# pscoro/JPEG-XL-Lossy-Image-Compression-Thesis

Hardware: AMD Instinct MI355X
Metric: MPix/s VarDCT encode @ d1.0, 8K RGB (higher is better)
Workload: dtype f32; 1 GPU; 8k 7680x4320 RGB8 (synth_rgb8), VarDCT d1 e7, cjxl defaults (JXG_FLAGS_CJXL_DEFAULTS: Gaborish + EPF + masking AQ), proposals=0, ans-coded, 1 frame(s) per step, 2 distinct frames cycled, streaming entry points (jxg_submit_rgb8_device / jxg_receive, one host thread); global_batch=1, parallelism=frame-dp1

## Files before the change

jpeg-xl-lossy-image-compression-thesis_amd/csrc/jxg_merge.hip:

```cpp
#include <float.h>

#include <cstdio>
#include <type_traits>

#include "jxg_device.h"
#include "jxg_kernels.h"
#include "jxg_lee_tables.h"

namespace jxg {

__constant__ float c_llf_p[4 * 8];
__constant__ float c_llf_ib[4 * 64];

constexpr int kMThreads = 256;
#ifndef JXG_MERGE_WPE
#define JXG_MERGE_WPE 4
#endif
#ifndef JXG_MERGE_WRITE_WPE
#define JXG_MERGE_WRITE_WPE 3
#endif
constexpr int kMS = 65;
constexpr int kMPlane = 64 * kMS;

template <int N>
constexpr int ilog2c() {
  return N <= 1 ? 0 : 1 + ilog2c<N / 2>();
}

typedef float f2 __attribute__((ext_vector_type(2)));

template <int N, class T>
__device__ __forceinline__ void lee(T* x) {
  if constexpr (N > 1) {
    constexpr int h = N / 2, l = ilog2c<N>();
    T a[h], b[h];
#pragma unroll
    for (int i = 0; i < h; i++) {
      a[i] = x[i] + x[N - 1 - i];
      b[i] = (x[i] - x[N - 1 - i]) * kLeeC[l][i];
    }
    lee<h>(a);
    lee<h>(b);
#pragma unroll
    for (int k = 0; k < h; k++) x[2 * k] = a[k];
#pragma unroll
    for (int k = 0; k < h - 1; k++) x[2 * k + 1] = b[k] + b[k + 1];
    x[N - 1] = b[h - 1];
  }
}
template <int N>
__device__ __forceinline__ void dct_from(const float* src, int st, float* x) {
#pragma unroll
  for (int k = 0; k < N; k++) x[k] = src[k * st];
  lee<N>(x);
  constexpr int l = ilog2c<N>();
#pragma unroll
  for (int k = 0; k < N; k++) x[k] = x[k] * kLeeS[l][k];
}
template <int N, class T>
__device__ __forceinline__ T dctN_first(T xi, T xm, int i, int h) {
  return h == 0 ? xi + xm : (xi - xm) * kLeeC[ilog2c<N>()][i];
}
template <int N, class T, class Out>
__device__ __forceinline__ void dctN_rest(T* t, int h, Out out) {
  constexpr int l = ilog2c<N>(), H = N / 2;
  lee<H>(t);
  if (h == 0) {
#pragma unroll
    for (int k = 0; k < H; k++) out(k, t[k] * kLeeS[l][2 * k]);
  } else {
#pragma unroll
    for (int k = 0; k < H - 1; k++) out(k, (t[k] + t[k + 1]) * kLeeS[l][2 * k + 1]);
    out(H - 1, t[H - 1] * kLeeS[l][N - 1]);
  }
}
template <class T>
__device__ __forceinline__ T dct64_first(T xi, T xm, int i, int h) {
  return dctN_first<64>(xi, xm, i, h);
}
template <class T, class Out>
__device__ __forceinline__ void dct64_rest(T* t, int h, Out out) {
  dctN_rest<64>(t, h, out);
}

#ifdef JXG_MERGE_PROFILE
__device__ unsigned long long g_mprof[16][8];
#define MPROF_MARK(k)                                                 \
  do {                                                                \
    if (!WRITE && threadIdx.x == 0) {                                 \
      const unsigned long long now_ = __builtin_readcyclecounter();   \
      if ((k) > 0) atomicAdd(&g_mprof[P.si][(k)], now_ - mprof_t0);   \
      mprof_t0 = now_;                                                \
    }                                                                 \
  } while (0)
#else
#define MPROF_MARK(k) \
  do {                \
  } while (0)
#endif
#ifdef JXG_MERGE_PROFILE
__device__ unsigned long long g_mzero[3][2];
#define MZERO_COUNT(ch, hit)                                                          \
  do {                                                                                \
    if ((int)(threadIdx.x & 63) == __ffsll((unsigned long long)__ballot(1)) - 1) {    \
      atomicAdd(&g_mzero[(ch)][0], 1ull);                                             \
      if (hit) atomicAdd(&g_mzero[(ch)][1], 1ull);                                    \
    }                                                                                 \
  } while (0)
#else
#define MZERO_COUNT(ch, hit) \
  do {                       \
  } while (0)
#endif

struct ShapeDesc {
  int type, lcy, lcx;
  float tmul;
};
constexpr ShapeDesc kShapes[kNumShapes] = {
    {6, 1, 0, 1.0f},   {7, 0, 1, 1.0f},   {4, 1, 1, 1.0f},
    {10, 2, 1, 1.02f}, {11, 1, 2, 1.02f}, {5, 2, 2, 1.03f},
    {19, 3, 2, 1.05f}, {20, 2, 3, 1.05f}, {18, 3, 3, 1.05f}};

__device__ __forceinline__ int bitlen_u(uint32_t v) { return 32 - __clz(v); }

struct MergeLds {
  float co[2 * kMPlane];
  float llf[3][64];
  float qsum[3][4][32];
  float btab[256];
  float vr3[32][3];
  int vbits[32];
  int vnz[32][3];
  int vraw[32];
  int valid[32];
  uint8_t braw[64];
  int any;
};
struct WriteLds : MergeLds {
  uint32_t ssrc[32];
  uint32_t sgb[32];
  float skc[2][32];
};
template <class L>
constexpr bool kIsWrite = std::is_same<L, WriteLds>::value;
__device__ __forceinline__ float& llf_at(MergeLds& S, int c, int b) { return S.llf[c][b]; }
__device__ __forceinline__ int pass_src(int pass, int lc) { return pass ? 2 : 1 - lc; }
__device__ __forceinline__ int pass_plane(int pass, int lc) { return pass ? 1 : lc; }
__device__ __forceinline__ constexpr int chan_plane(int ch) { return ch == 1 ? 0 : 1; }

struct Pass {
  int si, type, lcy, lcx, soff, ls, tx, ty, tile;
  float tmul;
  __device__ __forceinline__ int cy() const { return 1 << lcy; }
  __device__ __forceinline__ int cx() const { return 1 << lcx; }
  __device__ __forceinline__ int R() const { return 8 << lcy; }
  __device__ __forceinline__ int C() const { return 8 << lcx; }
  __device__ __forceinline__ int lR() const { return 3 + lcy; }
  __device__ __forceinline__ int lC() const { return 3 + lcx; }
  __device__ __forceinline__ int lGX() const { return 3 - lcx; }
  __device__ __forceinline__ int lNV() const { return 6 - lcx - lcy; }
  __device__ __forceinline__ int NV() const { return 1 << lNV(); }
  __device__ __forceinline__ int bx0(int v) const { return (v & ((1 << lGX()) - 1)) << lcx; }
  __device__ __forceinline__ int by0(int v) const { return (v >> lGX()) << lcy; }
  __device__ __forceinline__ int off(int v, int plane) const {
    return plane * kMPlane + by0(v) * 8 * kMS + bx0(v) * 8;
  }
};

#ifndef JXG_MERGE_CHUNK
#define JXG_MERGE_CHUNK 32
#endif
__device__ __forceinline__ bool decode_wg(const MergeArgs& a, int& tile, int& si) {
  constexpr int T = JXG_MERGE_CHUNK;
  const int b = blockIdx.x, x = b & 7, q = b >> 3;
  const int r = q % (kNumShapes * T);
  si = r / T;
  tile = ((q / (kNumShapes * T)) * T + r % T) * 8 + x;
  if (tile >= (int)a.ntiles) return false;
  if (a.tile_list) tile = (int)a.tile_list[tile];
  return true;
}

__device__ __forceinline__ Pass make_pass(const MergeArgs& a, int tile, int si) {
  Pass P;
  P.si = si;
  const ShapeDesc& D = kShapes[si];
  P.type = D.type;
  P.lcy = D.lcy;
  P.lcx = D.lcx;
  P.tmul = D.tmul;
  P.soff = kShapeOff[si];
  P.ls = max(D.lcy, D.lcx);
  P.tile = tile;
  P.tx = tile % (int)a.tiles_x;
  P.ty = tile / (int)a.tiles_x;
  return P;
}

template <int C>
__device__ __forceinline__ void load_row(const float* src, float* d) {
#pragma unroll
  for (int q = 0; q < C / 4; q++) {
    const float4 u = reinterpret_cast<const float4*>(src)[q];
    d[4 * q] = u.x;
    d[4 * q + 1] = u.y;
    d[4 * q + 2] = u.z;
    d[4 * q + 3] = u.w;
  }
}
template <int C, int NCH, class L>
__device__ __forceinline__ void row_pass(const MergeArgs& a, const Pass& P, L& S, int pass) {
  constexpr bool WRITE = kIsWrite<L>;
  const float* tsrc = a.xyb + (size_t)P.tile * (3 * 4096);
  const int R = P.R(), lvr = P.lNV() + P.lR();
  if constexpr (C == 64) {
    const int npairs = NCH * P.NV() * R / 2;
    const int n = ((npairs + 63) >> 6) << 7;
    for (int i = threadIdx.x; i < n; i += kMThreads) {
      const int h = (i >> 6) & 1, pp = ((i >> 7) << 6) | (i & 63), r = pp * 2;
      if (pp >= npairs) continue;
      const int c = r >> lvr, v = (r >> P.lR()) & (P.NV() - 1), y = r & (R - 1);
      if (!S.valid[v]) continue;
      const float* src0;
      if constexpr (WRITE) src0 = a.xyb + S.ssrc[v] + pass_src(pass, c) * 4096 + y * 64;
      else src0 = tsrc + pass_src(pass, c) * 4096 + (P.by0(v) * 8 + y) * 64;
      const float4* s0 = reinterpret_cast<const float4*>(src0);
      const float4* s1 = s0 + 16;
      f2 t[32];
#pragma unroll
      for (int q = 0; q < 8; q++) {
        const float4 a0 = s0[q], b0 = s0[15 - q], a1 = s1[q], b1 = s1[15 - q];
        const float fa0[4] = {a0.x, a0.y, a0.z, a0.w}, fb0[4] = {b0.x, b0.y, b0.z, b0.w};
        const float fa1[4] = {a1.x, a1.y, a1.z, a1.w}, fb1[4] = {b1.x, b1.y, b1.z, b1.w};
#pragma unroll
        for (int j = 0; j < 4; j++)
          t[4 * q + j] = dct64_first(f2{fa0[j], fa1[j]}, f2{fb0[3 - j], fb1[3 - j]}, 4 * q + j, h);
      }
      const int off = P.off(v, pass_plane(pass, c)) + y * kMS;
      dct64_rest(t, h, [&](int k, f2 o) {
        S.co[off + 2 * k + h] = o.x;
        S.co[off + kMS + 2 * k + h] = o.y;
      });
    }
  } else {
    constexpr int PER = (NCH * 4096 / C + kMThreads - 1) / kMThreads;
    const int nrows = NCH * P.NV() * R;
    const int lgx = P.lGX();
    auto row_of = [&](int rr, int& c, int& v, int& y) {
      c = rr >> lvr;
      const int i = rr & ((1 << lvr) - 1);
      y = (i >> lgx) & (R - 1);
      v = ((i >> (lgx + P.lR())) << lgx) | (i & ((1 << lgx) - 1));
    };
    float buf[PER][C];
#pragma unroll
    for (int k = 0; k < PER; k++) {
      const int r = threadIdx.x + k * kMThreads;
      if (r < nrows) {
        int c, v, y;
        row_of(r, c, v, y);
        if constexpr (WRITE)
          load_row<C>(a.xyb + S.ssrc[v] + pass_src(pass, c) * 4096 + y * 64, buf[k]);
        else
          load_row<C>(tsrc + pass_src(pass, c) * 4096 + (P.by0(v) * 8 + y) * 64 + P.bx0(v) * 8,
                      buf[k]);
      } else {
#pragma unroll
        for (int q = 0; q < C; q++) buf[k][q] = 0.0f;
      }
    }
    constexpr int l = ilog2c<C>();
#pragma unroll
    for (int k = 0; k < PER; k += 2) {
      const int r0 = threadIdx.x + k * kMThreads, r1 = r0 + kMThreads;
      if (r0 >= nrows) continue;
      int c0, v0, y0, c1, v1, y1;
      row_of(r0, c0, v0, y0);
      row_of(r1, c1, v1, y1);
      const bool ok0 = S.valid[v0], ok1 = k + 1 < PER && r1 < nrows && S.valid[v1];
      if (!ok0 && !ok1) continue;
      if (k + 1 < PER) {
        f2 x[C];
#pragma unroll
        for (int q = 0; q < C; q++) x[q] = f2{buf[k][q], buf[k + 1][q]};
        lee<C>(x);
        const int off0 = P.off(v0, pass_plane(pass, c0)) + y0 * kMS,
                  off1 = P.off(v1, pass_plane(pass, c1)) + y1 * kMS;
#pragma unroll
        for (int q = 0; q < C; q++) {
          const f2 o = x[q] * kLeeS[l][q];
          if (ok0) S.co[off0 + q] = o.x;
          if (ok1) S.co[off1 + q] = o.y;
        }
      } else {
        float* x = buf[k];
        lee<C>(x);
        const int off0 = P.off(v0, pass_plane(pass, c0)) + y0 * kMS;
#pragma unroll
        for (int q = 0; q < C; q++) S.co[off0 + q] = x[q] * kLeeS[l][q];
      }
    }
  }
}

template <int R, int NCH>
__device__ __forceinline__ void col_pass(const Pass& P, MergeLds& S, int pass) {
  constexpr int lR = ilog2c<R>(), nb = 64 / R, lnb = 6 - lR;
  constexpr int npairs = NCH * nb * 32;
  const int lGX = P.lGX(), lC = P.lC();
  auto col_of = [&](int pidx, int& off, bool& okA, bool& okB) {
    const int X = pidx & 31, band = (pidx >> 5) & (nb - 1), c = pidx >> (5 + lnb);
    off = pass_plane(pass, c) * kMPlane + band * R * kMS + X;
    okA = S.valid[(band << lGX) | (X >> lC)];
    okB = S.valid[(band << lGX) | ((X + 32) >> lC)];
  };
  if constexpr (R == 64 || (R >= 16 && npairs <= kMThreads / 2)) {
    constexpr int H = R / 2;
    constexpr int n = ((npairs + 63) >> 6) << 7;
    for (int i0 = 0; i0 < n; i0 += kMThreads) {
      const int i = i0 + threadIdx.x;
      const int h = (i >> 6) & 1, p = ((i >> 7) << 6) | (i & 63);
      int off = 0;
      bool okA = false, okB = false;
      if (p < npairs) col_of(p, off, okA, okB);
      const bool act = okA || okB;
      f2 o[H];
      if (act) {
        const float* q0 = S.co + off;
        f2 t[H];
#pragma unroll
        for (int j = 0; j < H; j++)
          t[j] = dctN_first<R>(f2{q0[j * kMS], q0[j * kMS + 32]},
                               f2{q0[(R - 1 - j) * kMS], q0[(R - 1 - j) * kMS + 32]}, j, h);
        dctN_rest<R>(t, h, [&](int k, f2 u) { o[k] = u; });
      }
      __syncthreads();
      if (act) {
#pragma unroll
        for (int k = 0; k < H; k++) {
          if (okA) S.co[off + (2 * k + h) * kMS] = o[k].x;
          if (okB) S.co[off + 32 + (2 * k + h) * kMS] = o[k].y;
        }
      }
    }
  } else {
    for (int p = threadIdx.x; p < npairs; p += kMThreads) {
      int off;
      bool okA, okB;
      col_of(p, off, okA, okB);
      if (!okA && !okB) continue;
      float* col = S.co + off;
      f2 o[R];
#pragma unroll
      for (int k = 0; k < R; k++) o[k] = f2{col[k * kMS], col[k * kMS + 32]};
      lee<R>(o);
#pragma unroll
      for (int k = 0; k < R; k++) {
        const f2 u = o[k] * kLeeS[lR][k];
        if (okA) col[k * kMS] = u.x;
        if (okB) col[k * kMS + 32] = u.y;
      }
    }
  }
}

template <int N>
__device__ __forceinline__ void load_f(const float* p, float* d) {
#pragma unroll
  for (int i = 0; i < N / 4; i++) {
    const float4 v = reinterpret_cast<const float4*>(p)[i];
    d[4 * i] = v.x;
    d[4 * i + 1] = v.y;
    d[4 * i + 2] = v.z;
    d[4 * i + 3] = v.w;
  }
}
template <int RPC>
struct QTab {
  static constexpr int NIT = RPC == 8 ? 2 : 1;
  float w[NIT][RPC], sd[NIT][RPC], iw[NIT][RPC];
};
__device__ __forceinline__ int qtab_index(const Pass& P, int ky, int x) {
  return P.soff + ((ky >> 2) * P.C() + x) * 4;
}
template <int RPC, bool WRITE, int CH>
__device__ __forceinline__ void load_qtab(const MergeArgs& a, const Pass& P, QTab<RPC>& T) {
  constexpr int STOT = kShapeOff[kNumShapes];
#pragma unroll
  for (int it = 0; it < QTab<RPC>::NIT; it++) {
    const int j = threadIdx.x + it * kMThreads;
    const int ch = j >> (P.lNV() + P.lC()), x = j & (P.C() - 1);
#pragma unroll
    for (int kk = 0; kk < RPC; kk += 4) {
      const int ti = qtab_index(P, ch * RPC + kk, x);
      load_f<4>(a.wk + (size_t)CH * STOT + ti, &T.w[it][kk]);
      if (!WRITE) load_f<4>(a.sdk + (size_t)CH * STOT + ti, &T.sd[it][kk]);
      if (CH == 1) load_f<4>(a.iwy + ti, &T.iw[it][kk]);
    }
  }
}
template <int M>
__device__ __forceinline__ uint32_t grp_xor(uint32_t v) {
  if constexpr (M == 1) return (uint32_t)__builtin_amdgcn_mov_dpp((int)v, 0xB1, 0xF, 0xF, false);
  if constexpr (M == 2) return (uint32_t)__builtin_amdgcn_mov_dpp((int)v, 0x4E, 0xF, 0xF, false);
  if constexpr (M == 4) {
    const int t = __builtin_amdgcn_mov_dpp((int)v, 0x1B, 0xF, 0xF, false);
    return (uint32_t)__builtin_amdgcn_mov_dpp(t, 0x141, 0xF, 0xF, false);
  }
  if constexpr (M == 8) {
    const int t = __builtin_amdgcn_mov_dpp((int)v, 0x141, 0xF, 0xF, false);
    return (uint32_t)__builtin_amdgcn_mov_dpp(t, 0x140, 0xF, 0xF, false);
  }
  if constexpr (M == 16) return (uint32_t)__builtin_amdgcn_ds_swizzle((int)v, 0x401F);
  if constexpr (M == 32) {
    const uint32_t lo = (uint32_t)__builtin_amdgcn_readlane((int)v, 0);
    const uint32_t hi = (uint32_t)__builtin_amdgcn_readlane((int)v, 32);
    return (threadIdx.x & 32) ? lo : hi;
  }
}
template <int M>
__device__ __forceinline__ void grp_step(float& cp, int& packed) {
  cp += __uint_as_float(grp_xor<M>(__float_as_uint(cp)));
  packed += (int)grp_xor<M>((uint32_t)packed);
}
__device__ __forceinline__ void group_all_reduce(float& cp, int& packed, int C) {
  grp_step<1>(cp, packed);
  grp_step<2>(cp, packed);
  grp_step<4>(cp, packed);
  if (C > 8) grp_step<8>(cp, packed);
  if (C > 16) grp_step<16>(cp, packed);
  if (C > 32) grp_step<32>(cp, packed);
}

template <int RPC, bool WRITE, int CH, class L>
__device__ __forceinline__ void quant_pass(const MergeArgs& a, const Pass& P, L& S, const QTab<RPC>& T) {
  static_assert(WRITE == kIsWrite<L>, "the write kernel's LDS carries the per-slot arrays");
  constexpr int cidx = CH == 1 ? 0 : (CH == 0 ? 1 : 2);
  constexpr bool ZERO = !WRITE && CH != 1;
  const int C = P.C(), NV = P.NV();
  float kc = 0.0f;
  if (!WRITE && CH != 1) {
    const float f = (float)a.cmap[(CH == 0 ? 0u : a.ntiles_all) + (uint32_t)P.tile];
    kc = CH == 0 ? f * (1.0f / 84.0f) : 1.0f + f * (1.0f / 84.0f);
  }
#pragma unroll
  for (int it = 0; it < QTab<RPC>::NIT; it++) {
    const int j = threadIdx.x + it * kMThreads;
    const int ch = j >> (P.lNV() + P.lC()), v = (j >> P.lC()) & (NV - 1), x = j & (C - 1);
    if (!S.valid[v]) continue;
    const int bx0 = P.bx0(v), by0 = P.by0(v);
    if constexpr (WRITE && CH != 1) kc = S.skc[CH == 0 ? 0 : 1][v];
    const float scale = (float)a.G * (float)S.vraw[v] / 65536.0f;
    float* cplane = S.co + P.off(v, chan_plane(CH)) + x;
    const float* yd = S.co + P.off(v, 0) + x;
    const float* w = T.w[it];
    const float* sd = T.sd[it];
    float iw[RPC];
    if (CH == 1) {
      const float inv_scale = 1.0f / scale;
#pragma unroll
      for (int kk = 0; kk < RPC; kk++) iw[kk] = T.iw[it][kk] * inv_scale;
    }
    uint16_t nat[RPC];
    if (WRITE) {
#pragma unroll
      for (int kk = 0; kk < RPC; kk += 4) {
        const uint2 u = *reinterpret_cast<const uint2*>(a.nat + qtab_index(P, ch * RPC + kk, x));
        nat[kk] = (uint16_t)u.x;
        nat[kk + 1] = (uint16_t)(u.x >> 16);
        nat[kk + 2] = (uint16_t)u.y;
        nat[kk + 3] = (uint16_t)(u.y >> 16);
      }
    }
    const bool llf_col = ch == 0 && x < P.cx();
    float cp = 0.0f;
    uint32_t eb8[2] = {0u, 0u};
    auto scaled = [&](int kk) {
      const int ky = ch * RPC + kk;
      const f2 coef = f2{cplane[ky * kMS], cplane[(ky + 1) * kMS]};
      if (WRITE && llf_col) {
        if (kk < P.cy()) llf_at(S, CH, (by0 + ky) * 8 + bx0 + x) = coef.x;
        if (kk + 1 < P.cy()) llf_at(S, CH, (by0 + ky + 1) * 8 + bx0 + x) = coef.y;
      }
      f2 rv = coef;
      if (CH != 1) rv = rv - f2{kc, kc} * f2{yd[ky * kMS], yd[(ky + 1) * kMS]};
      return rv * (f2{w[kk], w[kk + 1]} * f2{scale, scale});
    };
    f2 vqs[ZERO ? RPC / 2 : 1];
    if constexpr (ZERO) {
#pragma unroll
      for (int kk = 0; kk < RPC; kk += 2) vqs[kk >> 1] = scaled(kk);
    }
#pragma unroll
    for (int kk = 0; kk < RPC; kk += 2) {
      const int ky = ch * RPC + kk;
      f2 vq;
      if constexpr (ZERO) vq = vqs[kk >> 1];
      else vq = scaled(kk);
      if constexpr (ZERO) {
        const bool allz = !__any(!(fabsf(vq.x) < 0.58f) || !(fabsf(vq.y) < 0.58f));
        MZERO_COUNT(CH, allz);
        if (allz) {
          const f2 e = vq * f2{sd[kk], sd[kk + 1]};
          cp = fmaf(e.x, e.x, cp);
          cp = fmaf(e.y, e.y, cp);
          continue;
        }
      }
      float sqs[2], qfs[2];
#pragma unroll
      for (int h = 0; h < 2; h++) {
        const float vqh = h ? vq.y : vq.x;
        const float av = fabsf(vqh);
        qfs[h] = av < 0.58f ? 0.0f : floorf(fminf(av, 32767.0f) + 0.5f);
        sqs[h] = __builtin_copysignf(qfs[h], vqh);
      }
      if (CH == 1) {
        float adj[2];
#pragma unroll
        for (int h = 0; h < 2; h++) adj[h] = S.btab[min((int)qfs[h], 255)];
        if (__builtin_expect(__any(fmaxf(qfs[0], qfs[1]) >= 256.0f), 0)) {
#pragma unroll
          for (int h = 0; h < 2; h++)
            if (qfs[h] >= 256.0f) adj[h] = qfs[h] - 0.145f / qfs[h];
        }
#pragma unroll
        for (int h = 0; h < 2; h++) {
          const float a1 = __builtin_copysignf(adj[h], h ? vq.y : vq.x);
          cplane[(ky + h) * kMS] = a1 * iw[kk + h];
        }
      }
#pragma unroll
      for (int h = 0; h < 2; h++) {
        const float qf = qfs[h];
        eb8[kk >= 8] += __float_as_uint(qf) >> 23;
        if (WRITE) {
          const int qq = (int)sqs[h];
          const int p = nat[kk + h];
          const int sl = p >> 6;
          if constexpr (WRITE) {
            const size_t gb = (size_t)S.sgb[v] + (size_t)(sl >> P.lcx) * a.bxs + (sl & (P.cx() - 1));
            a.ac[(gb * 3 + CH) * 64 + (p & 63)] = (int16_t)qq;
          }
        }
      }
      if (!WRITE) {
        const f2 e = (vq - f2{sqs[0], sqs[1]}) * f2{sd[kk], sd[kk + 1]};
        cp = fmaf(e.x, e.x, cp);
        cp = fmaf(e.y, e.y, cp);
      }
    }
    const int nzc = (int)(eb8[0] / 127u) + (int)(eb8[1] / 127u);
    const int bits = 2 * (int)(eb8[0] + eb8[1]) - 250 * nzc;
    int packed = bits | nzc << 20;
    group_all_reduce(cp, packed, C);
    if (x == 0) {
      S.qsum[cidx][ch][v] = cp;
      if (packed & 0xFFFFF) atomicAdd(&S.vbits[v], packed & 0xFFFFF);
      if (packed >> 20) atomicAdd(&S.vnz[v][CH], packed >> 20);
    }
  }
}

template <bool WRITE, class L>
__device__ __forceinline__ void transform_quant(const MergeArgs& a, const Pass& P, L& S) {
#ifdef JXG_MERGE_PROFILE
  unsigned long long mprof_t0 = 0;
#endif
  MPROF_MARK(0);
  auto transform = [&](auto nch_tag, int pass) {
    constexpr int NCH = decltype(nch_tag)::value;
    switch (P.lcx) {
      case 0: row_pass<8, NCH>(a, P, S, pass); break;
      case 1: row_pass<16, NCH>(a, P, S, pass); break;
      case 2: row_pass<32, NCH>(a, P, S, pass); break;
      default: row_pass<64, NCH>(a, P, S, pass); break;
    }
    __syncthreads();
    switch (P.lcy) {
      case 0: col_pass<8, NCH>(P, S, pass); break;
      case 1: col_pass<16, NCH>(P, S, pass); break;
      case 2: col_pass<32, NCH>(P, S, pass); break;
      default: col_pass<64, NCH>(P, S, pass); break;
    }
  };
  transform(std::integral_constant<int, 2>(), 0);
  MPROF_MARK(1);
  auto quant_yx = [&](auto rpc_tag) {
    constexpr int RPC = decltype(rpc_tag)::value;
    {
      QTab<RPC> ty;
      load_qtab<RPC, WRITE, 1>(a, P, ty);
      __syncthreads();
      MPROF_MARK(2);
      quant_pass<RPC, WRITE, 1>(a, P, S, ty);
    }
    QTab<RPC> tx;
    load_qtab<RPC, WRITE, 0>(a, P, tx);
    quant_pass<RPC, WRITE, 0>(a, P, S, tx);
  };
  auto quant_b = [&](auto rpc_tag) {
    constexpr int RPC = decltype(rpc_tag)::value;
    QTab<RPC> tb;
    load_qtab<RPC, WRITE, 2>(a, P, tb);
    __syncthreads();
    quant_pass<RPC, WRITE, 2>(a, P, S, tb);
  };
  if (P.lcy == 0) quant_yx(std::integral_constant<int, 8>());
  else quant_yx(std::integral_constant<int, 16>());
  __syncthreads();
  MPROF_MARK(3);
  transform(std::integral_constant<int, 1>(), 1);
  if (P.lcy == 0) quant_b(std::integral_constant<int, 8>());
  else quant_b(std::integral_constant<int, 16>());
  __syncthreads();
  MPROF_MARK(4);
}

__device__ __forceinline__ float varblock_dist(const Pass& P, const MergeLds& S, int v) {
  const int nch = P.lcy == 0 ? 1 : P.R() >> 4;
  float pc[3];
#pragma unroll
  for (int ci = 0; ci < 3; ci++) {
    float t = S.qsum[ci][0][v];
    for (int ch = 1; ch < nch; ch++) t = t + S.qsum[ci][ch][v];
    pc[ci] = t;
  }
  return (pc[0] + pc[1]) + pc[2];
}

__device__ __forceinline__ void fill_btab(MergeLds& S) {
  for (int i = threadIdx.x; i < 256; i += kMThreads)
    S.btab[i] = i == 0 ? 0.0f : (i == 1 ? 1.0f - 0.07005449891748593f : (float)i - 0.145f / (float)i);
}
__device__ __forceinline__ void setup_varblocks(const MergeArgs& a, const Pass& P, MergeLds& S,
                                                int nbx, int nby) {
  const int t = threadIdx.x;
  if (t < 64) {
    const int lbx = t & 7, lby = t >> 3;
    const bool in = lbx < nbx && lby < nby;
    const size_t gb = (size_t)(P.ty * 8 + lby) * a.bxs + P.tx * 8 + lbx;
    S.braw[t] = in ? a.qf[gb] : 0;
  }
  if (t < 32) {
    const int v = t;
    bool ok = false;
    if (v < P.NV()) {
      const int bx0 = P.bx0(v), by0 = P.by0(v);
      const size_t gb0 = (size_t)(P.ty * 8 + by0) * a.bxs + P.tx * 8 + bx0;
      ok = (((bx0 >> P.ls) + 1) << P.ls) <= nbx && (((by0 >> P.ls) + 1) << P.ls) <= nby;
      if (ok && (a.proposals & 2u)) {
        S.vr3[v][0] = a.homog[gb0 * 3 + 0];
        S.vr3[v][1] = a.homog[gb0 * 3 + 1];
        S.vr3[v][2] = a.homog[gb0 * 3 + 2];
      }
    }
    S.valid[v] = ok;
    S.vraw[v] = 0;
    S.vbits[v] = 0;
    S.vnz[v][0] = S.vnz[v][1] = S.vnz[v][2] = 0;
  }
  fill_btab(S);
}
__device__ __forceinline__ void vraw_pass(const MergeArgs& a, const Pass& P, MergeLds& S) {
  (void)a;
  const int b = threadIdx.x;
  if (b < 64) {
    const int lbx = b & 7, lby = b >> 3;
    const int v = ((lby >> P.lcy) << P.lGX()) | (lbx >> P.lcx);
    if (v < P.NV() && S.valid[v]) atomicMax(&S.vraw[v], (int)S.braw[b] + 1);
  }
}
__device__ __forceinline__ void setup_slots(const MergeArgs& a, const Pass& P, WriteLds& S,
                                            const uint32_t* list, uint32_t first, uint32_t n) {
  (void)P;
  const int v = threadIdx.x;
  if (v < 32) {
    const bool ok = (uint32_t)v < n;
    uint32_t src = 0, gb0 = 0;
    float kx = 0.0f, kb = 0.0f;
    if (ok) {
      const uint32_t e = list[first + v], tile = e >> 6, by = (e >> 3) & 7u, bx = e & 7u;
      const uint32_t tx = tile % a.tiles_x, ty = tile / a.tiles_x;
      src = tile * (3u * 4096u) + by * (8u * 64u) + bx * 8u;
      gb0 = (ty * 8u + by) * a.bxs + tx * 8u + bx;
      kx = (float)a.cmap[tile] * (1.0f / 84.0f);
      kb = 1.0f + (float)a.cmap[a.ntiles_all + tile] * (1.0f / 84.0f);
    }
    S.ssrc[v] = src;
    S.sgb[v] = gb0;
    S.skc[0][v] = kx;
    S.skc[1][v] = kb;
    S.valid[v] = ok;
    S.vraw[v] = 0;
    S.vbits[v] = 0;
    S.vnz[v][0] = S.vnz[v][1] = S.vnz[v][2] = 0;
  }
  fill_btab(S);
}
__device__ __forceinline__ void vraw_slots(const MergeArgs& a, const Pass& P, WriteLds& S) {
  const int b = threadIdx.x;
  if (b < 64) {
    const int lbx = b & 7, lby = b >> 3;
    const int v = ((lby >> P.lcy) << P.lGX()) | (lbx >> P.lcx);
    if (v < P.NV() && S.valid[v]) {
      const size_t gb = (size_t)S.sgb[v] + (size_t)(lby & (P.cy() - 1)) * a.bxs + (lbx & (P.cx() - 1));
      atomicMax(&S.vraw[v], (int)a.qf[gb] + 1);
    }
  }
}

__device__ __forceinline__ int max_level(const MergeArgs& a) {
  return a.max_s >= 8 ? 3 : (a.max_s >= 4 ? 2 : 1);
}

__global__ __launch_bounds__(kMThreads) __attribute__((amdgpu_waves_per_eu(JXG_MERGE_WPE)))
void merge_eval_kernel(Batch<MergeArgs> bt_) {
  const MergeArgs& a = bt_.a[blockIdx.z];
  __shared__ __attribute__((aligned(16))) MergeLds S;
  if (blockIdx.x == 0 && threadIdx.x < kNumShapes) a.work[threadIdx.x] = 0;
  int tile, si;
  if (!decode_wg(a, tile, si)) return;
  const Pass P = make_pass(a, tile, si);
  if (P.ls > max_level(a)) return;
  const int nbx = min(8, (int)a.bxs - P.tx * 8), nby = min(8, (int)a.bys - P.ty * 8);
  if ((1 << P.ls) > nbx || (1 << P.ls) > nby) return;
#ifdef JXG_MERGE_PROFILE
  const unsigned long long t_setup = __builtin_readcyclecounter();
#endif
  setup_varblocks(a, P, S, nbx, nby);
  __syncthreads();
  vraw_pass(a, P, S);
#ifdef JXG_MERGE_PROFILE
  if (threadIdx.x == 0) atomicAdd(&g_mprof[P.si][5], __builtin_readcyclecounter() - t_setup);
#endif
  transform_quant<false>(a, P, S);
  const int v = threadIdx.x;
  if (v < P.NV() && S.valid[v]) {
    const float dist = varblock_dist(P, S, v);
    const int tb = bitlen_u((uint32_t)S.vnz[v][0]) + bitlen_u((uint32_t)S.vnz[v][1]) +
                   bitlen_u((uint32_t)S.vnz[v][2]);
    float e = ((float)(S.vbits[v] + tb) + 8.0f * dist) * P.tmul;
    if (a.proposals & 2u) e = hook_f(e, S.vr3[v][0], S.vr3[v][1], S.vr3[v][2]);
    a.cost[((size_t)tile * kNumShapes + si) * 32 + v] = e;
  }
}

constexpr int kResolveWaves = 16;
__device__ __forceinline__ void wave_sync_lds() {
  __builtin_amdgcn_fence(__ATOMIC_SEQ_CST, "wavefront");
  __builtin_amdgcn_wave_barrier();
}
__global__ __launch_bounds__(64 * kResolveWaves) void merge_resolve_kernel(Batch<MergeArgs> bt_) {
  const MergeArgs& a = bt_.a[blockIdx.z];
  __shared__ float sEntW[kResolveWaves][64];
  __shared__ uint8_t sAcsW[kResolveWaves][64];
  __shared__ uint32_t sCnt[kResolveWaves][kNumShapes];
  const int wv = threadIdx.x >> 6, t = threadIdx.x & 63;
  float* sEnt = sEntW[wv];
  uint8_t* sAcs = sAcsW[wv];
  const int idx = blockIdx.x * kResolveWaves + wv;
  int my = -1;
  int tile = 0;
  if (idx < (int)a.ntiles) {
    tile = a.tile_list ? (int)a.tile_list[idx] : idx;
    const int tx = tile % (int)a.tiles_x, ty = tile / (int)a.tiles_x;
    const int nbx = min(8, (int)a.bxs - tx * 8), nby = min(8, (int)a.bys - ty * 8);
    const int lbx = t & 7, lby = t >> 3;
    const bool in = lbx < nbx && lby < nby;
    const size_t gb = (size_t)(ty * 8 + lby) * a.bxs + tx * 8 + lbx;
    sEnt[t] = in ? a.ent[gb] : 0.0f;
    sAcs[t] = in ? a.acs[gb] : 0;
    wave_sync_lds();
    const float* cost = a.cost + (size_t)tile * kNumShapes * 32;
    for (int s = 2; s <= a.max_s && s <= nbx && s <= nby; s *= 2) {
      const int nr = 8 / s;
      const int full = s == 2 ? 2 : (s == 4 ? 5 : 8);
      const int tall = s == 2 ? 0 : (s == 4 ? 3 : 6);
      if (t < nr * nr) {
        const int rx = t % nr, ry = t / nr;
        if ((rx + 1) * s <= nbx && (ry + 1) * s <= nby) {
          float cur = 0.0f;
          for (int iy = 0; iy < s; iy++)
            for (int ix = 0; ix < s; ix++) cur += sEnt[(ry * s + iy) * 8 + rx * s + ix];
          const int vf = ry * nr + rx, vl = ry * (16 / s) + 2 * rx, vt = (2 * ry) * nr + rx;
          const float e0 = cost[full * 32 + vf];
          const float el = cost[tall * 32 + vl], er = cost[tall * 32 + vl + 1];
          const float etop = cost[(tall + 1) * 32 + vt], ebot = cost[(tall + 1) * 32 + vt + nr];
          const float et = el + er, ew = etop + ebot;
          float best = cur;
          int choice = 0;
          if (!(e0 >= best)) {
            best = e0;
            choice = 1;
          }
          if (!(et >= best)) {
            best = et;
            choice = 2;
          }
          if (!(ew >= best)) {
            best = ew;
            choice = 3;
          }
          for (int j = 0; choice && j < (choice == 1 ? 1 : 2); j++) {
            int sh, bx, by;
            float e;
            if (choice == 1) {
              sh = full, bx = rx * s, by = ry * s, e = e0;
            } else if (choice == 2) {
              sh = tall, bx = rx * s + j * (s / 2), by = ry * s, e = j ? er : el;
            } else {
              sh = tall + 1, bx = rx * s, by = ry * s + j * (s / 2), e = j ? ebot : etop;
            }
            const int cy = 1 << kShapes[sh].lcy, cx = 1 << kShapes[sh].lcx;
            for (int iy = 0; iy < cy; iy++)
              for (int ix = 0; ix < cx; ix++) {
                const int b = (by + iy) * 8 + bx + ix;
                sAcs[b] = (uint8_t)(kShapes[sh].type | ((iy | ix) ? 0x80 : 0));
                sEnt[b] = (iy | ix) ? 0.0f : e;
              }
          }
        }
      }
      wave_sync_lds();
    }
    if (in) {
      a.acs[gb] = sAcs[t];
// ... 148 lines not shown
#pragma unroll
    for (int j = kNumShapes - 1; j >= 0; j--) {
      const uint32_t np = (cnt[j] + kShapeSlots[j] - 1) / kShapeSlots[j];
      if (w >= start && w - start < np) {
        si = j;
        first = (w - start) * kShapeSlots[j];
        n = min((uint32_t)kShapeSlots[j], cnt[j] - first);
      }
      start += np;
    }
    write_pass(a, si, first, n, S);
    __syncthreads();
  }
}

__global__ __launch_bounds__(1024) void vb_list_kernel(Batch<VbArgs> bt_) {
  const VbArgs& a = bt_.a[blockIdx.z];
  __shared__ uint32_t sCnt[64 * 16];
  __shared__ uint32_t sWave[16];
  const uint32_t lg = blockIdx.x;
  if (a.lf_mine && !a.lf_mine[lg]) return;
  const uint32_t bx0 = (lg % a.lfxs) * 256, by0 = (lg / a.lfxs) * 256;
  const uint32_t bw = min(256u, a.bxs - bx0), bh = min(256u, a.bys - by0);
  const uint32_t n = bw * bh;
  const int lane = threadIdx.x & 63, wv = threadIdx.x >> 6;
  const uint64_t lt = (1ull << lane) - 1ull;
  const uint32_t dq = 1024u / bw, dr = 1024u % bw;
  const uint32_t y0 = threadIdx.x / bw, x0 = threadIdx.x % bw;
  auto step = [&](uint32_t& y, uint32_t& x) {
    x += dr;
    y += dq;
    if (x >= bw) {
      x -= bw;
      y++;
    }
  };
  uint64_t fl = 0;
  {
    uint32_t y = y0, x = x0;
#pragma unroll 16
    for (int k = 0; k < 64; k++) {
      const uint32_t i = (uint32_t)k * 1024 + threadIdx.x;
      if (i < n && !(a.acs[(size_t)(by0 + y) * a.bxs + bx0 + x] & 0x80)) fl |= 1ull << k;
      step(y, x);
    }
  }
  for (int k = 0; k < 64; k++) {
    const uint64_t bal = __ballot((fl >> k) & 1);
    if (lane == 0) sCnt[k * 16 + wv] = (uint32_t)__popcll(bal);
  }
  __syncthreads();
  const uint32_t v = sCnt[threadIdx.x];
  uint32_t incl = v;
#pragma unroll
  for (int d = 1; d < 64; d <<= 1) {
    const uint32_t t = __shfl_up(incl, d);
    if (lane >= d) incl += t;
  }
  if (lane == 63) sWave[wv] = incl;
  __syncthreads();
  uint32_t before = 0, total = 0;
  for (int w = 0; w < 16; w++) {
    before += w < wv ? sWave[w] : 0u;
    total += sWave[w];
  }
  sCnt[threadIdx.x] = before + incl - v;
  __syncthreads();
  uint32_t y = y0, x = x0;
  for (int k = 0; k < 64; k++) {
    const bool f = (fl >> k) & 1;
    const uint64_t bal = __ballot(f);
    if (f)
      a.vb[(size_t)lg * 65536 + sCnt[k * 16 + wv] + (uint32_t)__popcll(bal & lt)] =
          (uint32_t)((size_t)(by0 + y) * a.bxs + bx0 + x);
    step(y, x);
  }
  if (threadIdx.x == 0) a.count[lg] = total;
}

#ifdef JXG_MERGE_PROFILE
void dump_merge_profile() {
  unsigned long long h[16][8];
  if (hipMemcpyFromSymbol(h, HIP_SYMBOL(g_mprof), sizeof(h)) != hipSuccess) return;
  std::fprintf(stderr, "merge_eval cycles (thread 0 sums, Mcycles): shape setup rows+cols(Y,X) "
                       "qtab quantY+X B(rows,cols,quant)\n");
  for (int si = 0; si < kNumShapes; si++)
    std::fprintf(stderr, "  %dx%d %8.1f %8.1f %8.1f %8.1f %8.1f\n", 8 << kShapes[si].lcy,
                 8 << kShapes[si].lcx, h[si][5] / 1e6, h[si][1] / 1e6, h[si][2] / 1e6,
                 h[si][3] / 1e6, h[si][4] / 1e6);
  unsigned long long z[3][2];
  if (hipMemcpyFromSymbol(z, HIP_SYMBOL(g_mzero), sizeof(z)) != hipSuccess) return;
  for (int c = 0; c < 3; c++)
    std::fprintf(stderr, "quant_pass zero votes, channel %c: %llu of %llu row pairs\n", "XYB"[c],
                 z[c][1], z[c][0]);
}
#else
void dump_merge_profile() {}
#endif

hipError_t set_merge_constants(const float* llf_p, const float* llf_ib, hipStream_t s) {
  hipError_t e = hipMemcpyToSymbolAsync(HIP_SYMBOL(c_llf_p), llf_p, sizeof(float) * 4 * 8, 0,
                                        hipMemcpyHostToDevice, s);
  if (e == hipSuccess)
    e = hipMemcpyToSymbolAsync(HIP_SYMBOL(c_llf_ib), llf_ib, sizeof(float) * 4 * 64, 0,
                               hipMemcpyHostToDevice, s);
  const hipError_t e2 = hipStreamSynchronize(s);
  return e != hipSuccess ? e : e2;
}
hipError_t launch_merge(const MergeArgs* a, uint32_t k, hipStream_t s) {
  if (!k || !a[0].ntiles) return hipSuccess;
  const Batch<MergeArgs> b = make_batch(a, k);
  const uint32_t ntiles = a[0].ntiles;
  constexpr uint32_t T = JXG_MERGE_CHUNK;
  const uint32_t nwg = (((ntiles + 7) / 8 + T - 1) / T) * T * 8 * kNumShapes;
  hipLaunchKernelGGL(merge_eval_kernel, dim3(nwg, 1, k), dim3(kMThreads), 0, s, b);
  hipLaunchKernelGGL(merge_resolve_kernel, dim3((ntiles + kResolveWaves - 1) / kResolveWaves, 1, k),
                     dim3(64 * kResolveWaves), 0, s, b);
  const uint32_t nw = max(1u, min(a[0].nwrite / k, ntiles * (uint32_t)kNumShapes));
  hipLaunchKernelGGL(merge_write_kernel, dim3(nw, 1, k), dim3(kMThreads), 0, s, b);
  return hipGetLastError();
}
hipError_t launch_force_merge(const MergeArgs& a, hipStream_t s) {
  if (!a.ntiles || !a.force) return hipErrorInvalidValue;
  const hipError_t e = hipMemsetAsync(a.work, 0, kMergeWorkHead * sizeof(uint32_t), s);
  if (e != hipSuccess) return e;
  hipLaunchKernelGGL(force_list_kernel, dim3((a.ntiles + kResolveWaves - 1) / kResolveWaves),
                     dim3(64 * kResolveWaves), 0, s, a);
  const uint32_t nw = max(1u, min(a.nwrite, a.ntiles * (uint32_t)kNumShapes));
  hipLaunchKernelGGL(merge_write_kernel, dim3(nw, 1, 1), dim3(kMThreads), 0, s, make_batch(&a, 1));
  return hipGetLastError();
}
void launch_vb_list(const VbArgs* a, uint32_t k, uint32_t nlf, hipStream_t s) {
  if (k) hipLaunchKernelGGL(vb_list_kernel, dim3(nlf, 1, k), dim3(1024), 0, s, make_batch(a, k));
}

}
```

Before: 10790 MPix/s.

## Share row DCTs across block shapes of same width family in merge eval

```diff
diff --git a/jpeg-xl-lossy-image-compression-thesis_amd/csrc/jxg_merge.hip b/jpeg-xl-lossy-image-compression-thesis_amd/csrc/jxg_merge.hip
--- a/jpeg-xl-lossy-image-compression-thesis_amd/csrc/jxg_merge.hip
+++ b/jpeg-xl-lossy-image-compression-thesis_amd/csrc/jxg_merge.hip
@@ -14,7 +14,7 @@
 
 constexpr int kMThreads = 256;
 #ifndef JXG_MERGE_WPE
-#define JXG_MERGE_WPE 4
+#define JXG_MERGE_WPE 3
 #endif
 #ifndef JXG_MERGE_WRITE_WPE
 #define JXG_MERGE_WRITE_WPE 3
@@ -85,17 +85,17 @@
 
 #ifdef JXG_MERGE_PROFILE
 __device__ unsigned long long g_mprof[16][8];
-#define MPROF_MARK(k)                                                 \
+#define MPROF_MARK(si, k)                                             \
   do {                                                                \
-    if (!WRITE && threadIdx.x == 0) {                                 \
+    if (threadIdx.x == 0) {                                           \
       const unsigned long long now_ = __builtin_readcyclecounter();   \
-      if ((k) > 0) atomicAdd(&g_mprof[P.si][(k)], now_ - mprof_t0);   \
+      if ((k) > 0) atomicAdd(&g_mprof[(si)][(k)], now_ - mprof_t0);   \
       mprof_t0 = now_;                                                \
     }                                                                 \
   } while (0)
 #else
-#define MPROF_MARK(k) \
-  do {                \
+#define MPROF_MARK(si, k) \
+  do {                    \
   } while (0)
 #endif
 #ifdef JXG_MERGE_PROFILE
@@ -142,6 +142,18 @@
   uint32_t sgb[32];
   float skc[2][32];
 };
+struct EvalLds {
+  float co[3 * kMPlane];
+  float qsum[3][4][32];
+  float btab[256];
+  float vr3[32][3];
+  int vbits[32];
+  int vnz[32][3];
+  int vraw[32];
+  int valid[32];
+  uint8_t braw[64];
+};
+static_assert(sizeof(EvalLds) <= 42 * 1280, "three eval workgroups per CU: 42 LDS granules each");
 template <class L>
 constexpr bool kIsWrite = std::is_same<L, WriteLds>::value;
 __device__ __forceinline__ float& llf_at(MergeLds& S, int c, int b) { return S.llf[c][b]; }
@@ -304,14 +316,16 @@
   }
 }
 
-template <int R, int NCH>
-__device__ __forceinline__ void col_pass(const Pass& P, MergeLds& S, int pass) {
+template <int R, int NCH, bool B2 = false, class L>
+__device__ __forceinline__ void col_pass(const Pass& P, L& S, int pass) {
+  static_assert(!B2 || NCH == 1, "the out-of-place form is B's");
   constexpr int lR = ilog2c<R>(), nb = 64 / R, lnb = 6 - lR;
   constexpr int npairs = NCH * nb * 32;
+  constexpr int dst = B2 ? -kMPlane : 0;
   const int lGX = P.lGX(), lC = P.lC();
   auto col_of = [&](int pidx, int& off, bool& okA, bool& okB) {
     const int X = pidx & 31, band = (pidx >> 5) & (nb - 1), c = pidx >> (5 + lnb);
-    off = pass_plane(pass, c) * kMPlane + band * R * kMS + X;
+    off = (B2 ? 2 : pass_plane(pass, c)) * kMPlane + band * R * kMS + X;
     okA = S.valid[(band << lGX) | (X >> lC)];
     okB = S.valid[(band << lGX) | ((X + 32) >> lC)];
   };
@@ -335,12 +349,12 @@
                                f2{q0[(R - 1 - j) * kMS], q0[(R - 1 - j) * kMS + 32]}, j, h);
         dctN_rest<R>(t, h, [&](int k, f2 u) { o[k] = u; });
       }
-      __syncthreads();
+      if constexpr (!B2) __syncthreads();
       if (act) {
 #pragma unroll
         for (int k = 0; k < H; k++) {
-          if (okA) S.co[off + (2 * k + h) * kMS] = o[k].x;
-          if (okB) S.co[off + 32 + (2 * k + h) * kMS] = o[k].y;
+          if (okA) S.co[off + dst + (2 * k + h) * kMS] = o[k].x;
+          if (okB) S.co[off + dst + 32 + (2 * k + h) * kMS] = o[k].y;
         }
       }
     }
@@ -358,8 +372,8 @@
 #pragma unroll
       for (int k = 0; k < R; k++) {
         const f2 u = o[k] * kLeeS[lR][k];
-        if (okA) col[k * kMS] = u.x;
-        if (okB) col[k * kMS + 32] = u.y;
+        if (okA) col[dst + k * kMS] = u.x;
+        if (okB) col[dst + k * kMS + 32] = u.y;
       }
     }
   }
@@ -479,9 +493,11 @@
     auto scaled = [&](int kk) {
       const int ky = ch * RPC + kk;
       const f2 coef = f2{cplane[ky * kMS], cplane[(ky + 1) * kMS]};
-      if (WRITE && llf_col) {
-        if (kk < P.cy()) llf_at(S, CH, (by0 + ky) * 8 + bx0 + x) = coef.x;
-        if (kk + 1 < P.cy()) llf_at(S, CH, (by0 + ky + 1) * 8 + bx0 + x) = coef.y;
+      if constexpr (WRITE) {
+        if (llf_col) {
+          if (kk < P.cy()) llf_at(S, CH, (by0 + ky) * 8 + bx0 + x) = coef.x;
+          if (kk + 1 < P.cy()) llf_at(S, CH, (by0 + ky + 1) * 8 + bx0 + x) = coef.y;
+        }
       }
       f2 rv = coef;
       if (CH != 1) rv = rv - f2{kc, kc} * f2{yd[ky * kMS], yd[(ky + 1) * kMS]};
@@ -565,10 +581,6 @@
 
 template <bool WRITE, class L>
 __device__ __forceinline__ void transform_quant(const MergeArgs& a, const Pass& P, L& S) {
-#ifdef JXG_MERGE_PROFILE
-  unsigned long long mprof_t0 = 0;
-#endif
-  MPROF_MARK(0);
   auto transform = [&](auto nch_tag, int pass) {
     constexpr int NCH = decltype(nch_tag)::value;
     switch (P.lcx) {
@@ -586,14 +598,12 @@
     }
   };
   transform(std::integral_constant<int, 2>(), 0);
-  MPROF_MARK(1);
   auto quant_yx = [&](auto rpc_tag) {
     constexpr int RPC = decltype(rpc_tag)::value;
     {
       QTab<RPC> ty;
       load_qtab<RPC, WRITE, 1>(a, P, ty);
       __syncthreads();
-      MPROF_MARK(2);
       quant_pass<RPC, WRITE, 1>(a, P, S, ty);
     }
     QTab<RPC> tx;
@@ -610,15 +620,13 @@
   if (P.lcy == 0) quant_yx(std::integral_constant<int, 8>());
   else quant_yx(std::integral_constant<int, 16>());
   __syncthreads();
-  MPROF_MARK(3);
   transform(std::integral_constant<int, 1>(), 1);
   if (P.lcy == 0) quant_b(std::integral_constant<int, 8>());
   else quant_b(std::integral_constant<int, 16>());
   __syncthreads();
-  MPROF_MARK(4);
-}
-
-__device__ __forceinline__ float varblock_dist(const Pass& P, const MergeLds& S, int v) {
+}
+
+__device__ __forceinline__ float varblock_dist(const Pass& P, const EvalLds& S, int v) {
   const int nch = P.lcy == 0 ? 1 : P.R() >> 4;
   float pc[3];
 #pragma unroll
@@ -630,19 +638,25 @@
   return (pc[0] + pc[1]) + pc[2];
 }
 
-__device__ __forceinline__ void fill_btab(MergeLds& S) {
+template <class L>
+__device__ __forceinline__ void fill_btab(L& S) {
   for (int i = threadIdx.x; i < 256; i += kMThreads)
     S.btab[i] = i == 0 ? 0.0f : (i == 1 ? 1.0f - 0.07005449891748593f : (float)i - 0.145f / (float)i);
 }
-__device__ __forceinline__ void setup_varblocks(const MergeArgs& a, const Pass& P, MergeLds& S,
-                                                int nbx, int nby) {
+__device__ __forceinline__ void setup_tile(const MergeArgs& a, EvalLds& S, int tx, int ty, int nbx,
+                                           int nby) {
   const int t = threadIdx.x;
   if (t < 64) {
     const int lbx = t & 7, lby = t >> 3;
     const bool in = lbx < nbx && lby < nby;
-    const size_t gb = (size_t)(P.ty * 8 + lby) * a.bxs + P.tx * 8 + lbx;
+    const size_t gb = (size_t)(ty * 8 + lby) * a.bxs + tx * 8 + lbx;
     S.braw[t] = in ? a.qf[gb] : 0;
   }
+  fill_btab(S);
+}
+__device__ __forceinline__ void setup_varblocks(const MergeArgs& a, const Pass& P, EvalLds& S,
+                                                int nbx, int nby) {
+  const int t = threadIdx.x;
   if (t < 32) {
     const int v = t;
     bool ok = false;
@@ -661,9 +675,8 @@
     S.vbits[v] = 0;
     S.vnz[v][0] = S.vnz[v][1] = S.vnz[v][2] = 0;
   }
-  fill_btab(S);
-}
-__device__ __forceinline__ void vraw_pass(const MergeArgs& a, const Pass& P, MergeLds& S) {
+}
+__device__ __forceinline__ void vraw_pass(const MergeArgs& a, const Pass& P, EvalLds& S) {
   (void)a;
   const int b = threadIdx.x;
   if (b < 64) {
@@ -715,35 +728,248 @@
   return a.max_s >= 8 ? 3 : (a.max_s >= 4 ? 2 : 1);
 }
 
+__device__ __forceinline__ int family_first(int f) { return f ? 3 * f - 2 : 0; }
+__device__ __forceinline__ int family_count(int f) { return f == 0 ? 1 : (f == 3 ? 2 : 3); }
+
+template <int LCX>
+__device__ __forceinline__ void family_rows(const MergeArgs& a, int tile, EvalLds& S, int nbx,
+                                            int nby, float (&hv)[32]) {
+  constexpr int C = 8 << LCX;
+  constexpr int LM = LCX ? LCX : 1;
+  auto need = [&](int Y, int gx) {
+    const int bx0 = gx << LCX, by = Y >> 3;
+    return (((bx0 >> LM) + 1) << LM) <= nbx && (((by >> LM) + 1) << LM) <= nby;
+  };
+  const float* tsrc = a.xyb + (size_t)tile * (3 * 4096);
+  float* bdst = S.co + 2 * kMPlane;
+  if constexpr (C == 64) {
+    const int i = threadIdx.x, h = (i >> 6) & 1, row = ((i >> 7) << 6) | (i & 63);
+    const int c = row >> 6, Y = row & 63;
+    auto half_row = [&](const float* src, float* t) {
+      const float4* s0 = reinterpret_cast<const float4*>(src);
+#pragma unroll
+      for (int q = 0; q < 8; q++) {
+        const float4 a0 = s0[q], b0 = s0[15 - q];
+        const float fa0[4] = {a0.x, a0.y, a0.z, a0.w}, fb0[4] = {b0.x, b0.y, b0.z, b0.w};
+#pragma unroll
+        for (int j = 0; j < 4; j++) t[4 * q + j] = dct64_first(fa0[j], fb0[3 - j], 4 * q + j, h);
+      }
+    };
+    if (!need(Y, 0)) return;
+    {
+      float t[32];
+      half_row(tsrc + pass_src(0, c) * 4096 + Y * 64, t);
+      dct64_rest(t, h, [&](int k, float o) { hv[k] = o; });
+    }
+    if (i < 128) {
+      float t[32];
+      half_row(tsrc + 2 * 4096 + Y * 64, t);
+      dct64_rest(t, h, [&](int k, float o) { bdst[Y * kMS + 2 * k + h] = o; });
+    }
+  } else {
+    constexpr int l = ilog2c<C>(), lgx = 3 - LCX, lch = 9 - LCX;
+    constexpr int PER = (2 << lch) / kMThreads;
+    constexpr int NB = 1 << lch, PB = (NB + kMThreads - 1) / kMThreads;
+    auto seg_of = [&](int r, int& c, int& Y, int& gx) {
+      c = r >> lch;
+      const int i = r & (NB - 1);
+      gx = i & ((1 << lgx) - 1);
+      Y = i >> lgx;
+    };
+    float buf[PER][C], bb[PB][C];
+#pragma unroll
+    for (int k = 0; k < PER; k++) {
+      int c, Y, gx;
+      seg_of(threadIdx.x + k * kMThreads, c, Y, gx);
+      load_row<C>(tsrc + pass_src(0, c) * 4096 + Y * 64 + gx * C, buf[k]);
+    }
+#pragma unroll
+    for (int k = 0; k < PB; k++) {
+      const int r = threadIdx.x + k * kMThreads;
+      if (r < NB) {
+        int c, Y, gx;
+        seg_of(r, c, Y, gx);
+        load_row<C>(tsrc + 2 * 4096 + Y * 64 + gx * C, bb[k]);
+      } else {
+#pragma unroll
+        for (int q = 0; q < C; q++) bb[k][q] = 0.0f;
+      }
+    }
+#pragma unroll
+    for (int k = 0; k < PER; k += 2) {
+      int c0, Y0, gx0, c1 = 0, Y1 = 0, gx1 = 0;
+      seg_of(threadIdx.x + k * kMThreads, c0, Y0, gx0);
+      if (k + 1 < PER) seg_of(threadIdx.x + (k + 1) * kMThreads, c1, Y1, gx1);
+      const bool n0 = need(Y0, gx0), n1 = k + 1 < PER && need(Y1, gx1);
+      if (!n0 && !n1) continue;
+      if constexpr (PER >= 2) {
+        f2 x[C];
+#pragma unroll
+        for (int q = 0; q < C; q++) x[q] = f2{buf[k][q], buf[k + 1][q]};
+        lee<C>(x);
+#pragma unroll
+        for (int q = 0; q < C; q++) {
+          const f2 o = x[q] * kLeeS[l][q];
+          hv[k * C + q] = o.x;
+          hv[(k + 1) * C + q] = o.y;
+        }
+      } else {
+        float* x = buf[k];
+        lee<C>(x);
+#pragma unroll
+        for (int q = 0; q < C; q++) hv[q] = x[q] * kLeeS[l][q];
+      }
+    }
+#pragma unroll
+    for (int k = 0; k < PB; k += 2) {
+      const int r0 = threadIdx.x + k * kMThreads, r1 = r0 + kMThreads;
+      if (r0 >= NB) continue;
+      int c0, Y0, gx0, c1 = 0, Y1 = 0, gx1 = 0;
+      seg_of(r0, c0, Y0, gx0);
+      if (k + 1 < PB) seg_of(r1, c1, Y1, gx1);
+      const bool n0 = need(Y0, gx0), n1 = k + 1 < PB && r1 < NB && need(Y1, gx1);
+      if (!n0 && !n1) continue;
+      if constexpr (PB >= 2) {
+        f2 x[C];
+#pragma unroll
+        for (int q = 0; q < C; q++) x[q] = f2{bb[k][q], bb[k + 1][q]};
+        lee<C>(x);
+        float* d0 = bdst + Y0 * kMS + gx0 * C;
+        float* d1 = bdst + Y1 * kMS + gx1 * C;
+#pragma unroll
+        for (int q = 0; q < C; q++) {
+          const f2 o = x[q] * kLeeS[l][q];
+          if (n0) d0[q] = o.x;
+          if (n1) d1[q] = o.y;
+        }
+      } else {
+        float* x = bb[k];
+        lee<C>(x);
+        float* d0 = bdst + Y0 * kMS + gx0 * C;
+#pragma unroll
+        for (int q = 0; q < C; q++) d0[q] = x[q] * kLeeS[l][q];
+      }
+    }
+  }
+}
+
+template <int LCX>
+__device__ __forceinline__ void family_writeout(const Pass& P, EvalLds& S, const float (&hv)[32]) {
+  constexpr int C = 8 << LCX;
+  if constexpr (C == 64) {
+    const int i = threadIdx.x, h = (i >> 6) & 1, row = ((i >> 7) << 6) | (i & 63);
+    const int c = row >> 6, Y = row & 63;
+    if (!S.valid[Y >> P.lR()]) return;
+    float* d = S.co + pass_plane(0, c) * kMPlane + Y * kMS + h;
+#pragma unroll
+    for (int k = 0; k < 32; k++) d[2 * k] = hv[k];
+  } else {
+    constexpr int lgx = 3 - LCX, lch = 9 - LCX, PER = (2 << lch) / kMThreads;
+#pragma unroll
+    for (int k = 0; k < PER; k++) {
+      const int r = threadIdx.x + k * kMThreads;
+      const int c = r >> lch, i = r & ((1 << lch) - 1), gx = i & ((1 << lgx) - 1), Y = i >> lgx;
+      if (!S.valid[((Y >> P.lR()) << lgx) | gx]) continue;
+      float* d = S.co + pass_plane(0, c) * kMPlane + Y * kMS + gx * C;
+#pragma unroll
+      for (int q = 0; q < C; q++) d[q] = hv[k * C + q];
+    }
+  }
+}
+
 __global__ __launch_bounds__(kMThreads) __attribute__((amdgpu_waves_per_eu(JXG_MERGE_WPE)))
 void merge_eval_kernel(Batch<MergeArgs> bt_) {
   const MergeArgs& a = bt_.a[blockIdx.z];
-  __shared__ __attribute__((aligned(16))) MergeLds S;
+  __shared__ __attribute__((aligned(16))) EvalLds S;
   if (blockIdx.x == 0 && threadIdx.x < kNumShapes) a.work[threadIdx.x] = 0;
-  int tile, si;
-  if (!decode_wg(a, tile, si)) return;
-  const Pass P = make_pass(a, tile, si);
-  if (P.ls > max_level(a)) return;
-  const int nbx = min(8, (int)a.bxs - P.tx * 8), nby = min(8, (int)a.bys - P.ty * 8);
-  if ((1 << P.ls) > nbx || (1 << P.ls) > nby) return;
+  int tile, si0;
+  if (!decode_wg(a, tile, si0)) return;
+  const int fam = kShapes[si0].lcx;
+  if (si0 != family_first(fam)) return;
+  const int lm = max(fam, 1), maxl = max_level(a);
+  const int tx = tile % (int)a.tiles_x, ty = tile / (int)a.tiles_x;
+  const int nbx = min(8, (int)a.bxs - tx * 8), nby = min(8, (int)a.bys - ty * 8);
+  if (lm > maxl || (1 << lm) > nbx || (1 << lm) > nby) return;
 #ifdef JXG_MERGE_PROFILE
-  const unsigned long long t_setup = __builtin_readcyclecounter();
+  unsigned long long mprof_t0 = 0;
 #endif
-  setup_varblocks(a, P, S, nbx, nby);
-  __syncthreads();
-  vraw_pass(a, P, S);
-#ifdef JXG_MERGE_PROFILE
-  if (threadIdx.x == 0) atomicAdd(&g_mprof[P.si][5], __builtin_readcyclecounter() - t_setup);
-#endif
-  transform_quant<false>(a, P, S);
-  const int v = threadIdx.x;
-  if (v < P.NV() && S.valid[v]) {
-    const float dist = varblock_dist(P, S, v);
-    const int tb = bitlen_u((uint32_t)S.vnz[v][0]) + bitlen_u((uint32_t)S.vnz[v][1]) +
-                   bitlen_u((uint32_t)S.vnz[v][2]);
-    float e = ((float)(S.vbits[v] + tb) + 8.0f * dist) * P.tmul;
-    if (a.proposals & 2u) e = hook_f(e, S.vr3[v][0], S.vr3[v][1], S.vr3[v][2]);
-    a.cost[((size_t)tile * kNumShapes + si) * 32 + v] = e;
+  MPROF_MARK(si0, 0);
+  setup_tile(a, S, tx, ty, nbx, nby);
+  float hv[32];
+#pragma unroll
+  for (int q = 0; q < 32; q++) hv[q] = 0.0f;
+  switch (fam) {
+    case 0: family_rows<0>(a, tile, S, nbx, nby, hv); break;
+    case 1: family_rows<1>(a, tile, S, nbx, nby, hv); break;
+    case 2: family_rows<2>(a, tile, S, nbx, nby, hv); break;
+    default: family_rows<3>(a, tile, S, nbx, nby, hv); break;
+  }
+  MPROF_MARK(si0, 6);
+  for (int si = si0; si < si0 + family_count(fam); si++) {
+    const Pass P = make_pass(a, tile, si);
+    if (P.ls > maxl || (1 << P.ls) > nbx || (1 << P.ls) > nby) continue;
+    MPROF_MARK(si, 0);
+    setup_varblocks(a, P, S, nbx, nby);
+    __syncthreads();
+    vraw_pass(a, P, S);
+    switch (fam) {
+      case 0: family_writeout<0>(P, S, hv); break;
+      case 1: family_writeout<1>(P, S, hv); break;
+      case 2: family_writeout<2>(P, S, hv); break;
+      default: family_writeout<3>(P, S, hv); break;
+    }
+    __syncthreads();
+    MPROF_MARK(si, 5);
+    switch (P.lcy) {
+      case 0: col_pass<8, 2>(P, S, 0); break;
+      case 1: col_pass<16, 2>(P, S, 0); break;
+      case 2: col_pass<32, 2>(P, S, 0); break;
+      default: col_pass<64, 2>(P, S, 0); break;
+    }
+    MPROF_MARK(si, 1);
+    auto quant_yx = [&](auto rpc_tag) {
+      constexpr int RPC = decltype(rpc_tag)::value;
+      {
+        QTab<RPC> ty_;
+        load_qtab<RPC, false, 1>(a, P, ty_);
+        __syncthreads();
+        MPROF_MARK(si, 2);
+        quant_pass<RPC, false, 1>(a, P, S, ty_);
+      }
+      QTab<RPC> tx_;
+      load_qtab<RPC, false, 0>(a, P, tx_);
+      quant_pass<RPC, false, 0>(a, P, S, tx_);
+    };
+    auto quant_b = [&](auto rpc_tag) {
+      constexpr int RPC = decltype(rpc_tag)::value;
+      QTab<RPC> tb;
+      load_qtab<RPC, false, 2>(a, P, tb);
+      __syncthreads();
+      quant_pass<RPC, false, 2>(a, P, S, tb);
+    };
+    if (P.lcy == 0) quant_yx(std::integral_constant<int, 8>());
+    else quant_yx(std::integral_constant<int, 16>());
+    __syncthreads();
+    MPROF_MARK(si, 3);
+    switch (P.lcy) {
+      case 0: col_pass<8, 1, true>(P, S, 1); break;
+      case 1: col_pass<16, 1, true>(P, S, 1); break;
+      case 2: col_pass<32, 1, true>(P, S, 1); break;
+      default: col_pass<64, 1, true>(P, S, 1); break;
+    }
+    if (P.lcy == 0) quant_b(std::integral_constant<int, 8>());
+    else quant_b(std::integral_constant<int, 16>());
+    __syncthreads();
+    MPROF_MARK(si, 4);
+    const int v = threadIdx.x;
+    if (v < P.NV() && S.valid[v]) {
+      const float dist = varblock_dist(P, S, v);
+      const int tb = bitlen_u((uint32_t)S.vnz[v][0]) + bitlen_u((uint32_t)S.vnz[v][1]) +
+                     bitlen_u((uint32_t)S.vnz[v][2]);
+      float e = ((float)(S.vbits[v] + tb) + 8.0f * dist) * P.tmul;
+      if (a.proposals & 2u) e = hook_f(e, S.vr3[v][0], S.vr3[v][1], S.vr3[v][2]);
+      a.cost[((size_t)tile * kNumShapes + si) * 32 + v] = e;
+    }
   }
 }
 
@@ -1058,11 +1284,11 @@
 void dump_merge_profile() {
   unsigned long long h[16][8];
   if (hipMemcpyFromSymbol(h, HIP_SYMBOL(g_mprof), sizeof(h)) != hipSuccess) return;
-  std::fprintf(stderr, "merge_eval cycles (thread 0 sums, Mcycles): shape setup rows+cols(Y,X) "
-                       "qtab quantY+X B(rows,cols,quant)\n");
+  std::fprintf(stderr, "merge_eval cycles (thread 0 sums, Mcycles): shape rows(family) "
+                       "setup+writeout cols(Y,X) qtab quantY+X B(cols,quant)\n");
   for (int si = 0; si < kNumShapes; si++)
-    std::fprintf(stderr, "  %dx%d %8.1f %8.1f %8.1f %8.1f %8.1f\n", 8 << kShapes[si].lcy,
-                 8 << kShapes[si].lcx, h[si][5] / 1e6, h[si][1] / 1e6, h[si][2] / 1e6,
+    std::fprintf(stderr, "  %dx%d %8.1f %8.1f %8.1f %8.1f %8.1f %8.1f\n", 8 << kShapes[si].lcy,
+                 8 << kShapes[si].lcx, h[si][6] / 1e6, h[si][5] / 1e6, h[si][1] / 1e6, h[si][2] / 1e6,
                  h[si][3] / 1e6, h[si][4] / 1e6);
   unsigned long long z[3][2];
   if (hipMemcpyFromSymbol(z, HIP_SYMBOL(g_mzero), sizeof(z)) != hipSuccess) return;
```

Measured after the change: 10980 MPix/s, median of 6. 1.02x the previous value.
